# henriChevreux/distillation_trajectories

Measured on AMD Instinct MI355X. Metric: trajectory-timesteps/sec (B×T U-Net fwd) at 16×16 T=50, higher is better.
Workload: dtype f32 (fp32-accurate; convolutions: exact 3-plane bf16 operand split on bf16 MFMA with fp32 accumulate, or native fp32 MFMA, chosen per layer)

## Files before the change

### distillation_trajectories_amd/csrc/dt_conv_strip.hip

```cpp
#include <mutex>
#include <type_traits>

#include "dt_conv_epilogue.h"

namespace dt {

extern __shared__ __attribute__((aligned(16))) __bf16 strip_lds[];

template <int BM, int BN, int KC = 1, int WK = 1>
__global__ __launch_bounds__(256, KC == 1 ? 3 : 2) void conv_strip_bf16x6_kernel(const ConvParams p) {
  constexpr int WN = WK > 1 ? BN / 64 : (BM == 256 ? 1 : 2), WM = 4 / (WN * WK), NT = 256;
  constexpr int MI = BM / (32 * WM), NI = BN / (32 * WN);
  constexpr int KW = KC / WK;
  static_assert(KC % WK == 0 && MI * 32 * WM == BM && NI * 32 * WN == BN && (WK == 1 || (MI == 2 && NI == 2)), "wave layout");
  constexpr int PLANE_B = BN * 16, STAGE_B = 3 * PLANE_B;
  constexpr int AP = BM == 256 ? 3 : (KC == 4 ? 1 : 2);
  const int halo = strip_halo(p.W, BM);
  const int R = BM + 2 * halo;
  const int RZ = (R + 7) & ~7;
  const int PLANE_A = (RZ + 8) * 16;
  __bf16 *As = strip_lds;
  __bf16 *Bs = strip_lds + KC * 3 * PLANE_A;

  const int tid = threadIdx.x, lane = tid & 63;
  const int wave = __builtin_amdgcn_readfirstlane(tid >> 6);
  const int wk = wave % WK, wm = (wave / WK) / WN, wn = (wave / WK) % WN;
  const int half = lane >> 5, l31 = lane & 31;
  const int m0 = blockIdx.x * BM, n0 = blockIdx.y * BN;
  const int HW = p.H * p.W;
  const int CC = p.cin_p >> 4;

  bool s_in[AP], s_ok[AP], s_core[AP];
  int s_off[AP], s_off2[AP], s_offb[AP], s_lds[AP];
#pragma unroll
  for (int i = 0; i < AP; ++i) {
    const int item = tid + i * NT;
    const int srow = item >> 1, hh = item & 1;
    const int m = m0 - halo + srow;
    s_in[i] = item < 2 * R;
    s_ok[i] = s_in[i] && m >= 0 && m < p.M;
    s_core[i] = s_ok[i] && srow >= halo && srow < halo + BM;
    const int mm = s_ok[i] ? m : 0;
    s_off[i] = mm * p.cin_p + hh * 8;
    s_off2[i] = mm * p.cin2_p + hh * 8;
    s_offb[i] = mm * p.b_stride + hh * 8;
    s_lds[i] = srow * 16 + ((hh ^ ((srow >> 3) & 1)) << 3);
  }
  constexpr bool B_ALL = WK > 1 && BN * 4 == NT;
  constexpr int NB = B_ALL ? KC * 3 / 2 : KC * 3, SB = B_ALL ? 2 : 1;
  static_assert(!B_ALL || (KC * 3) % 2 == 0, "weight staging");
  const bool b_thread = B_ALL || tid < BN * 2;
  const int bt = B_ALL ? (tid & (BN * 2 - 1)) : tid, bsub = B_ALL ? tid / (BN * 2) : 0;
  const size_t w_plane = (size_t)p.n_p * 16;
  const __bf16 *wbase = reinterpret_cast<const __bf16 *>(p.w) + (size_t)n0 * 16 + bt * 8 + bsub * w_plane;
  const __bf16 *wbase2 = reinterpret_cast<const __bf16 *>(p.w2) + (size_t)n0 * 16 + bt * 8 + bsub * w_plane;
  const int b_lds = bsub * PLANE_B + bt * 8;

  int a_row[MI];
  unsigned a_mask[MI];
#pragma unroll
  for (int mi = 0; mi < MI; ++mi) {
    const int row_i = wm * (MI * 32) + mi * 32 + l31;
    const int m = m0 + row_i;
    a_row[mi] = row_i + halo;
    unsigned mask = 0;
    if (m < p.M) {
      const int rem = m % HW;
      const int y = rem / p.W, x = rem - y * p.W;
#pragma unroll
      for (int t = 0; t < 9; ++t) {
        const int yy = y + t / 3 - 1, xx = x + t % 3 - 1;
        if (yy >= 0 && yy < p.H && xx >= 0 && xx < p.W) mask |= 1u << t;
      }
    }
    a_mask[mi] = mask;
  }
  int b_frag[NI];
#pragma unroll
  for (int ni = 0; ni < NI; ++ni) {
    const int row = wn * (NI * 32) + ni * 32 + l31;
    b_frag[ni] = row * 16 + ((half ^ ((row >> 3) & 1)) << 3);
  }

  f32x16 acc[MI][NI];
#pragma unroll
  for (int mi = 0; mi < MI; ++mi)
#pragma unroll
    for (int ni = 0; ni < NI; ++ni)
#pragma unroll
      for (int r = 0; r < 16; ++r) acc[mi][ni][r] = 0.f;

  const int n_main = (CC + p.splits * KC - 1) / (p.splits * KC);
  const int cc0 = blockIdx.z * n_main * KC;
  const int CC2 = p.cin2_p >> 4;
  const int n_chunks = n_main + (p.in2 ? (CC2 + KC - 1) / KC : 0);

  f32x4 sa0[KC][AP], sa1[KC][AP];
  u32x4 rb[NB];
  auto load_strip = [&](int ch) __attribute__((always_inline)) {
#pragma unroll
    for (int kk = 0; kk < KC; ++kk)
#pragma unroll
    for (int i = 0; i < AP; ++i) {
      sa0[kk][i] = f32x4{0.f, 0.f, 0.f, 0.f}; sa1[kk][i] = sa0[kk][i];
      if (ch < n_main) {
        const int cc = cc0 + ch * KC + kk;
        if (s_ok[i] && cc < CC) {
          const float *src = (p.in_b && cc >= p.cc_a) ? p.in_b + s_offb[i] + (cc - p.cc_a) * 16 : p.in + s_off[i] + cc * 16;
          sa0[kk][i] = *reinterpret_cast<const f32x4 *>(src);
          sa1[kk][i] = *reinterpret_cast<const f32x4 *>(src + 4);
        }
      } else if (s_core[i] && (ch - n_main) * KC + kk < CC2) {
        const int c2 = (ch - n_main) * KC + kk;
        const float *src = (p.in2_b && c2 >= p.cc_a) ? p.in2_b + s_offb[i] + (c2 - p.cc_a) * 16 : p.in2 + s_off2[i] + c2 * 16;
        sa0[kk][i] = *reinterpret_cast<const f32x4 *>(src);
        sa1[kk][i] = *reinterpret_cast<const f32x4 *>(src + 4);
      }
    }
  };
  auto write_strip = [&]() __attribute__((always_inline)) {
#pragma unroll
    for (int kk = 0; kk < KC; ++kk)
#pragma unroll
    for (int i = 0; i < AP; ++i)
      if (s_in[i]) {
        bf16x8 p1, p2, p3;
        split8(sa0[kk][i], sa1[kk][i], p1, p2, p3);
        __bf16 *A = As + kk * 3 * PLANE_A;
        *reinterpret_cast<bf16x8 *>(A + s_lds[i]) = p1;
        *reinterpret_cast<bf16x8 *>(A + PLANE_A + s_lds[i]) = p2;
        *reinterpret_cast<bf16x8 *>(A + 2 * PLANE_A + s_lds[i]) = p3;
      }
  };
  const size_t tap_stride = (size_t)p.ccw * 3 * w_plane, group_stride = (size_t)KC * 3 * w_plane;
  const __bf16 *wrun = wbase + (size_t)cc0 * 3 * w_plane;
  enum { ADV_NONE = 0, ADV_TAP, ADV_GROUP, ADV_SKIP0, ADV_SKIP };
  auto load_b = [&](int adv) __attribute__((always_inline)) {
    if (adv == ADV_TAP) wrun += tap_stride;
    else if (adv == ADV_GROUP) wrun = wrun - 8 * tap_stride + group_stride;
    else if (adv == ADV_SKIP0) wrun = wbase2;
    else if (adv == ADV_SKIP) wrun += group_stride;
    if (b_thread) {
#pragma unroll
      for (int i = 0; i < NB; ++i)
        rb[i] = *reinterpret_cast<const u32x4 *>(wrun + (SB * i) * w_plane);
    }
  };
  auto write_b = [&](int stage) __attribute__((always_inline)) {
    if (b_thread) {
      __bf16 *B = Bs + stage * KC * STAGE_B;
#pragma unroll
      for (int i = 0; i < NB; ++i) *reinterpret_cast<u32x4 *>(B + (SB * i) * PLANE_B + b_lds) = rb[i];
    }
  };

  constexpr bool DB = WK > 1;
  bf16x8 fbn[KW][NI][3];
  auto load_bd = [&](int adv) __attribute__((always_inline)) {
    if (adv == ADV_TAP) wrun += tap_stride;
    else if (adv == ADV_GROUP) wrun = wrun - 8 * tap_stride + group_stride;
    else if (adv == ADV_SKIP0) wrun = wbase2;
    else if (adv == ADV_SKIP) wrun += group_stride;
    const __bf16 *wt = wrun - (bt * 8 + bsub * w_plane);
#pragma unroll
    for (int kw = 0; kw < KW; ++kw)
#pragma unroll
      for (int ni = 0; ni < NI; ++ni)
#pragma unroll
        for (int pl = 0; pl < 3; ++pl)
          fbn[kw][ni][pl] = *reinterpret_cast<const bf16x8 *>(wt + ((wk * KW + kw) * 3 + pl) * w_plane + b_frag[ni]);
  };

  load_strip(0);
  if (DB) load_bd(ADV_NONE); else load_b(ADV_NONE);
  if (tid < 48 * KC) *reinterpret_cast<u32x4 *>(As + (tid >> 4) * PLANE_A + RZ * 16 + (tid & 15) * 8) = u32x4{0u, 0u, 0u, 0u};
  write_strip();
  if (!DB) write_b(0);
  __syncthreads();

  int step = 0;
  bool stage_next_strip = true;
  auto do_step = [&](auto TT, int ch, bool first_tap, bool last_tap, bool next_chunk, int adv) __attribute__((always_inline)) {
    constexpr int tt = decltype(TT)::value;
    const bool more = !last_tap || next_chunk;
    if (first_tap && next_chunk && stage_next_strip) load_strip(ch + 1);
    bf16x8 fbc[KW][NI][3];
    if (DB) {
#pragma unroll
      for (int kw = 0; kw < KW; ++kw)
#pragma unroll
        for (int ni = 0; ni < NI; ++ni)
#pragma unroll
          for (int pl = 0; pl < 3; ++pl) fbc[kw][ni][pl] = fbn[kw][ni][pl];
      if (more) load_bd(adv);
    } else if (more) load_b(adv);
    {
      int wv = p.W;
      asm volatile("" : "+s"(wv));
      const int shift = (tt / 3 - 1) * wv + (tt % 3 - 1);
      int a_e[MI];
#pragma unroll
      for (int mi = 0; mi < MI; ++mi) {
        int row0 = a_row[mi];
        asm volatile("" : "+v"(row0));
        const int srow = row0 + shift;
        const int lrow = ((a_mask[mi] >> tt) & 1u) ? srow : RZ + (srow & 7);
        a_e[mi] = lrow * 16 + ((half ^ ((srow >> 3) & 1)) << 3);
      }
#pragma unroll
      for (int kw = 0; kw < KW; ++kw) {
        const int kk = wk * KW + kw;
        const __bf16 *A = As + kk * 3 * PLANE_A;
        const __bf16 *B = Bs + ((step & 1) * KC + kk) * STAGE_B;
        bf16x8 fb[NI][3];
#pragma unroll
        for (int ni = 0; ni < NI; ++ni)
#pragma unroll
          for (int pl = 0; pl < 3; ++pl)
            fb[ni][pl] = DB ? fbc[kw][ni][pl] : *reinterpret_cast<const bf16x8 *>(B + pl * PLANE_B + b_frag[ni]);
#pragma unroll
        for (int mi = 0; mi < MI; ++mi) {
          bf16x8 fa[3];
#pragma unroll
          for (int pl = 0; pl < 3; ++pl)
            fa[pl] = *reinterpret_cast<const bf16x8 *>(A + pl * PLANE_A + a_e[mi]);
#pragma unroll
          for (int ni = 0; ni < NI; ++ni) {
            f32x16 c = acc[mi][ni];
            c = __builtin_amdgcn_mfma_f32_32x32x16_bf16(fa[2], fb[ni][0], c, 0, 0, 0);
            c = __builtin_amdgcn_mfma_f32_32x32x16_bf16(fa[1], fb[ni][1], c, 0, 0, 0);
            c = __builtin_amdgcn_mfma_f32_32x32x16_bf16(fa[0], fb[ni][2], c, 0, 0, 0);
            c = __builtin_amdgcn_mfma_f32_32x32x16_bf16(fa[1], fb[ni][0], c, 0, 0, 0);
            c = __builtin_amdgcn_mfma_f32_32x32x16_bf16(fa[0], fb[ni][1], c, 0, 0, 0);
            c = __builtin_amdgcn_mfma_f32_32x32x16_bf16(fa[0], fb[ni][0], c, 0, 0, 0);
            acc[mi][ni] = c;
          }
        }
      }
    }
    if (!DB && more) write_b((step + 1) & 1);
    const bool restage = last_tap && next_chunk && stage_next_strip;
    if (restage) {
      __syncthreads();
      write_strip();
    }
    if (!DB || restage) __syncthreads();
    ++step;
  };

  constexpr bool DIRECT = MI * KW <= 2 && KC >= 2;
  f32x4 ga0[KW][MI][2], ga1[KW][MI][2];
  const int n_skip = p.in2 ? (CC2 + KC - 1) / KC : 0;
  auto load_a = [&](f32x4 (&g)[KW][MI][2], int s2) __attribute__((always_inline)) {
#pragma unroll
    for (int kw = 0; kw < KW; ++kw)
#pragma unroll
      for (int mi = 0; mi < MI; ++mi) {
        const int c2 = s2 * KC + wk * KW + kw;
        const int m = m0 + wm * (MI * 32) + mi * 32 + l31;
        g[kw][mi][0] = f32x4{0.f, 0.f, 0.f, 0.f}; g[kw][mi][1] = g[kw][mi][0];
        if (m < p.M && c2 < CC2) {
          const float *src = (p.in2_b && c2 >= p.cc_a) ? p.in2_b + (size_t)m * p.b_stride + (c2 - p.cc_a) * 16 + half * 8
                                                       : p.in2 + (size_t)m * p.cin2_p + c2 * 16 + half * 8;
          g[kw][mi][0] = *reinterpret_cast<const f32x4 *>(src);
          g[kw][mi][1] = *reinterpret_cast<const f32x4 *>(src + 4);
        }
      }
  };
  auto skip_step = [&](f32x4 (&g)[KW][MI][2], int s2) __attribute__((always_inline)) {
    const bool more = s2 + 1 < n_skip;
    bf16x8 fbc[KW][NI][3];
    if (DB) {
#pragma unroll
      for (int kw = 0; kw < KW; ++kw)
#pragma unroll
        for (int ni = 0; ni < NI; ++ni)
#pragma unroll
          for (int pl = 0; pl < 3; ++pl) fbc[kw][ni][pl] = fbn[kw][ni][pl];
      if (more) load_bd(ADV_SKIP);
    } else if (more) load_b(ADV_SKIP);
#pragma unroll
    for (int kw = 0; kw < KW; ++kw) {
      const int kk = wk * KW + kw;
      const __bf16 *B = Bs + ((step & 1) * KC + kk) * STAGE_B;
      bf16x8 fb[NI][3];
#pragma unroll
      for (int ni = 0; ni < NI; ++ni)
#pragma unroll
        for (int pl = 0; pl < 3; ++pl) fb[ni][pl] = DB ? fbc[kw][ni][pl] : *reinterpret_cast<const bf16x8 *>(B + pl * PLANE_B + b_frag[ni]);
#pragma unroll
      for (int mi = 0; mi < MI; ++mi) {
        bf16x8 fa[3];
        split8(g[kw][mi][0], g[kw][mi][1], fa[0], fa[1], fa[2]);
#pragma unroll
        for (int ni = 0; ni < NI; ++ni) {
          f32x16 c = acc[mi][ni];
          c = __builtin_amdgcn_mfma_f32_32x32x16_bf16(fa[2], fb[ni][0], c, 0, 0, 0);
          c = __builtin_amdgcn_mfma_f32_32x32x16_bf16(fa[1], fb[ni][1], c, 0, 0, 0);
          c = __builtin_amdgcn_mfma_f32_32x32x16_bf16(fa[0], fb[ni][2], c, 0, 0, 0);
          c = __builtin_amdgcn_mfma_f32_32x32x16_bf16(fa[1], fb[ni][0], c, 0, 0, 0);
          c = __builtin_amdgcn_mfma_f32_32x32x16_bf16(fa[0], fb[ni][1], c, 0, 0, 0);
          c = __builtin_amdgcn_mfma_f32_32x32x16_bf16(fa[0], fb[ni][0], c, 0, 0, 0);
          acc[mi][ni] = c;
        }
      }
    }
    if (s2 + 2 < n_skip) load_a(g, s2 + 2);
    if (!DB) {
      if (more) write_b((step + 1) & 1);
      __syncthreads();
    }
    ++step;
  };

  const int prio_grp = ((blockIdx.x + gridDim.x * (blockIdx.y + gridDim.y * blockIdx.z)) >> 8) & 1;
  const bool use_prio = gridDim.x * gridDim.y * gridDim.z <= 512;
  for (int ch = 0; ch < n_main; ++ch) {
    if (use_prio) {
      if ((ch ^ prio_grp) & 1) __builtin_amdgcn_s_setprio(1);
      else __builtin_amdgcn_s_setprio(0);
    }
    const bool next_chunk = ch + 1 < ((WK > 1 && p.in2) ? n_main : n_chunks);
    if (DIRECT && WK == 1 && p.in2 && ch + 1 == n_main) {
      stage_next_strip = false;
      load_a(ga0, 0);
      if (n_skip > 1) load_a(ga1, 1);
    }
    do_step(std::integral_constant<int, 0>{}, ch, true, false, next_chunk, ADV_TAP);
    do_step(std::integral_constant<int, 1>{}, ch, false, false, next_chunk, ADV_TAP);
    do_step(std::integral_constant<int, 2>{}, ch, false, false, next_chunk, ADV_TAP);
    do_step(std::integral_constant<int, 3>{}, ch, false, false, next_chunk, ADV_TAP);
    do_step(std::integral_constant<int, 4>{}, ch, false, false, next_chunk, ADV_TAP);
    do_step(std::integral_constant<int, 5>{}, ch, false, false, next_chunk, ADV_TAP);
    do_step(std::integral_constant<int, 6>{}, ch, false, false, next_chunk, ADV_TAP);
    do_step(std::integral_constant<int, 7>{}, ch, false, false, next_chunk, ADV_TAP);
    do_step(std::integral_constant<int, 8>{}, ch, false, true, next_chunk, ch + 1 < n_main ? ADV_GROUP : ADV_SKIP0);
    if (ch + 1 == n_main && p.in2) {
      if constexpr (WK == 1) {
        conv_midpoint<MI, NI>(p, acc, n0, wn, l31);
      } else {
        constexpr int P = BN + 4, COPY = WM * 32 * P;
        float *red = reinterpret_cast<float *>(strip_lds);
#pragma unroll
        for (int mi = 0; mi < MI; ++mi) {
          if (mi || DB) __syncthreads();
#pragma unroll
          for (int ni = 0; ni < NI; ++ni)
#pragma unroll
            for (int r = 0; r < 16; ++r)
              red[wk * COPY + (wm * 32 + 4 * half + (r & 3) + 8 * (r >> 2)) * P + wn * (NI * 32) + ni * 32 + l31] = acc[mi][ni][r];
          __syncthreads();
#pragma unroll
          for (int ni = 0; ni < NI; ++ni)
#pragma unroll
            for (int r = 0; r < 16; ++r) {
              const float *src = red + (wm * 32 + 4 * half + (r & 3) + 8 * (r >> 2)) * P + wn * (NI * 32) + ni * 32 + l31;
              float v = src[0];
#pragma unroll
              for (int c = 1; c < WK; ++c) v += src[c * COPY];
              acc[mi][ni][r] = wk == 0 ? v : 0.f;
            }
        }
        if (wk == 0) conv_midpoint<MI, NI>(p, acc, n0, wn, l31);
        __syncthreads();
        if (DB) load_bd(ADV_SKIP0); else load_b(ADV_SKIP0);
        if (DIRECT) {
          load_a(ga0, 0);
          if (n_skip > 1) load_a(ga1, 1);
        } else {
          load_strip(n_main);
          if (tid < 48 * KC) *reinterpret_cast<u32x4 *>(As + (tid >> 4) * PLANE_A + RZ * 16 + (tid & 15) * 8) = u32x4{0u, 0u, 0u, 0u};
          write_strip();
        }
        if (!DB) write_b(step & 1);
        __syncthreads();
      }
    }
  }
  __builtin_amdgcn_s_setprio(0);
  if (DIRECT) {
    for (int s2 = 0; s2 < n_skip; s2 += 2) {
      skip_step(ga0, s2);
      if (s2 + 1 < n_skip) skip_step(ga1, s2 + 1);
    }
  } else {
    for (int ch = n_main; ch < n_chunks; ++ch)
      do_step(std::integral_constant<int, 4>{}, ch, true, true, ch + 1 < n_chunks, ADV_SKIP);
  }
  conv_epilogue<MI, NI, WM, WK>(p, acc, reinterpret_cast<float *>(strip_lds), m0, n0, wm, wn, half, l31, wk);
}

int launch_conv_strip(const ConvParams &p_in, hipStream_t s) {
  ConvParams p = p_in;
  const int bm = p.bm, bn = p.bn, kind = p.kind;
  const int kc = strip_kc(kind, bm, bn);
  dim3 grid((p.M + bm - 1) / bm, p.n_p / bn, p.splits);
  size_t lds = strip_lds_bytes(p.W, bm, bn, kind);
  p.dup_stage2 = 0;
  if (p.n_dup == 2 && p.pool_out) {
    const size_t rows1 = bm == 256 || kc == 4 || (kind == KIND_STRIPK && bm == 128) ? 128 : 64;
    const size_t rows2 = bm == 256 ? 128 : (bm == 128 ? 64 : 32);
    const size_t need = (rows1 + (kind == KIND_STRIPK ? rows2 : rows1)) * (bn + 4) * sizeof(float);
    if (need <= strip_lds_limit(kind)) {
      p.dup_stage2 = 1;
      if (need > lds) lds = need;
    }
  }
  if (kind != KIND_STRIP) {
    static std::once_flag attr_once;
    static int attr_status = DT_OK;
    std::call_once(attr_once, [] {
      const void *fns[8] = {reinterpret_cast<const void *>(&conv_strip_bf16x6_kernel<64, 128, 2, 2>),
                            reinterpret_cast<const void *>(&conv_strip_bf16x6_kernel<64, 64, 4, 4>),
                            reinterpret_cast<const void *>(&conv_strip_bf16x6_kernel<128, 64, 2, 2>),
                            reinterpret_cast<const void *>(&conv_strip_bf16x6_kernel<256, 64, 2>),
                            reinterpret_cast<const void *>(&conv_strip_bf16x6_kernel<128, 128, 2>),
                            reinterpret_cast<const void *>(&conv_strip_bf16x6_kernel<128, 64, 2>),
                            reinterpret_cast<const void *>(&conv_strip_bf16x6_kernel<64, 128, 2>),
                            reinterpret_cast<const void *>(&conv_strip_bf16x6_kernel<64, 64, 2>)};
      for (const void *f : fns) {
        const hipError_t e = hipFuncSetAttribute(f, hipFuncAttributeMaxDynamicSharedMemorySize, 98304);
        if (e != hipSuccess) attr_status = (int)e;
      }
    });
    if (attr_status != DT_OK) return attr_status;
    if (kind == KIND_STRIPK && bn == 128) conv_strip_bf16x6_kernel<64, 128, 2, 2><<<grid, 256, lds, s>>>(p);
    else if (kind == KIND_STRIPK && bm == 64) conv_strip_bf16x6_kernel<64, 64, 4, 4><<<grid, 256, lds, s>>>(p);
    else if (kind == KIND_STRIPK) conv_strip_bf16x6_kernel<128, 64, 2, 2><<<grid, 256, lds, s>>>(p);
    else if (bm == 256) conv_strip_bf16x6_kernel<256, 64, 2><<<grid, 256, lds, s>>>(p);
    else if (bm == 128 && bn == 128) conv_strip_bf16x6_kernel<128, 128, 2><<<grid, 256, lds, s>>>(p);
    else if (bm == 128) conv_strip_bf16x6_kernel<128, 64, 2><<<grid, 256, lds, s>>>(p);
    else if (bn == 128) conv_strip_bf16x6_kernel<64, 128, 2><<<grid, 256, lds, s>>>(p);
    else conv_strip_bf16x6_kernel<64, 64, 2><<<grid, 256, lds, s>>>(p);
    DT_LAUNCH_CHECK();
    return DT_OK;
  }
  if (bm == 256) conv_strip_bf16x6_kernel<256, 64><<<grid, 256, lds, s>>>(p);
  else if (bm == 128 && bn == 128) conv_strip_bf16x6_kernel<128, 128><<<grid, 256, lds, s>>>(p);
  else if (bm == 128) conv_strip_bf16x6_kernel<128, 64><<<grid, 256, lds, s>>>(p);
  else if (bn == 128) conv_strip_bf16x6_kernel<64, 128><<<grid, 256, lds, s>>>(p);
  else conv_strip_bf16x6_kernel<64, 64><<<grid, 256, lds, s>>>(p);
  DT_LAUNCH_CHECK();
  return DT_OK;
}

}
```

Before: 353,700.

## Double-buffer A strip in split-K strip conv, staging one item per tap

For the split-K (WK>1) strip convolution variants, the A input strip becomes a two-buffer ring in LDS. Next-chunk strip items are loaded and split into bf16 planes one item per tap, interleaved with the MFMA work, instead of loaded at the first tap and written behind an extra barrier at chunk end. The weight pointer is recomputed per tile without per-thread offsets, and the split-K reduction for the skip input moves out of the chunk loop. The cost is roughly double the A-strip LDS footprint, with the dynamic LDS cap raised to 160KB for these kernels, which can lower occupancy.

```diff
diff --git a/distillation_trajectories_amd/csrc/dt_conv_strip.hip b/distillation_trajectories_amd/csrc/dt_conv_strip.hip
--- a/distillation_trajectories_amd/csrc/dt_conv_strip.hip
+++ b/distillation_trajectories_amd/csrc/dt_conv_strip.hip
@@ -132,6 +132,32 @@
         *reinterpret_cast<bf16x8 *>(A + 2 * PLANE_A + s_lds[i]) = p3;
       }
   };
+  constexpr int NS = KC * AP;
+  f32x4 st0, st1;
+  auto load_item = [&](auto J, int ch) __attribute__((always_inline)) {
+    constexpr int kk = decltype(J)::value / AP, i = decltype(J)::value % AP;
+    const int cc = cc0 + ch * KC + kk, ccl = cc < CC ? cc : CC - 1;
+    const bool ok = s_ok[i] && cc < CC, from_b = p.in_b && ccl >= p.cc_a;
+    const float *base = from_b ? p.in_b + (ccl - p.cc_a) * 16 : p.in + ccl * 16;
+    unsigned off = s_off[i], offb = s_offb[i];
+    asm volatile("" : "+v"(off), "+v"(offb));
+    const float *src = base + (from_b ? offb : off);
+    const f32x4 v0 = *reinterpret_cast<const f32x4 *>(src), v1 = *reinterpret_cast<const f32x4 *>(src + 4);
+    const f32x4 z = {0.f, 0.f, 0.f, 0.f};
+    st0 = ok ? v0 : z;
+    st1 = ok ? v1 : z;
+  };
+  auto write_item = [&](auto J, int buf) __attribute__((always_inline)) {
+    constexpr int kk = decltype(J)::value / AP, i = decltype(J)::value % AP;
+    if (s_in[i]) {
+      bf16x8 p1, p2, p3;
+      split8(st0, st1, p1, p2, p3);
+      __bf16 *A = As + (buf * KC + kk) * 3 * PLANE_A;
+      *reinterpret_cast<bf16x8 *>(A + s_lds[i]) = p1;
+      *reinterpret_cast<bf16x8 *>(A + PLANE_A + s_lds[i]) = p2;
+      *reinterpret_cast<bf16x8 *>(A + 2 * PLANE_A + s_lds[i]) = p3;
+    }
+  };
   const size_t tap_stride = (size_t)p.ccw * 3 * w_plane, group_stride = (size_t)KC * 3 * w_plane;
   const __bf16 *wrun = wbase + (size_t)cc0 * 3 * w_plane;
   enum { ADV_NONE = 0, ADV_TAP, ADV_GROUP, ADV_SKIP0, ADV_SKIP };
@@ -155,25 +181,31 @@
   };
 
   constexpr bool DB = WK > 1;
+  static_assert(!DB || NS <= 8, "strip items staged one per tap");
   bf16x8 fbn[KW][NI][3];
+  const __bf16 *wtile = DB ? reinterpret_cast<const __bf16 *>(p.w) + (size_t)n0 * 16 + (size_t)cc0 * 3 * w_plane : nullptr;
   auto load_bd = [&](int adv) __attribute__((always_inline)) {
-    if (adv == ADV_TAP) wrun += tap_stride;
-    else if (adv == ADV_GROUP) wrun = wrun - 8 * tap_stride + group_stride;
-    else if (adv == ADV_SKIP0) wrun = wbase2;
-    else if (adv == ADV_SKIP) wrun += group_stride;
-    const __bf16 *wt = wrun - (bt * 8 + bsub * w_plane);
+    if (adv == ADV_TAP) wtile += tap_stride;
+    else if (adv == ADV_GROUP) wtile = wtile - 8 * tap_stride + group_stride;
+    else if (adv == ADV_SKIP0) wtile = reinterpret_cast<const __bf16 *>(p.w2) + (size_t)n0 * 16;
+    else if (adv == ADV_SKIP) wtile += group_stride;
 #pragma unroll
     for (int kw = 0; kw < KW; ++kw)
 #pragma unroll
-      for (int ni = 0; ni < NI; ++ni)
+      for (int ni = 0; ni < NI; ++ni) {
+        unsigned off = b_frag[ni];
+        asm volatile("" : "+v"(off));
 #pragma unroll
         for (int pl = 0; pl < 3; ++pl)
-          fbn[kw][ni][pl] = *reinterpret_cast<const bf16x8 *>(wt + ((wk * KW + kw) * 3 + pl) * w_plane + b_frag[ni]);
+          fbn[kw][ni][pl] = *reinterpret_cast<const bf16x8 *>(wtile + ((wk * KW + kw) * 3 + pl) * w_plane + off);
+      }
   };
 
   load_strip(0);
   if (DB) load_bd(ADV_NONE); else load_b(ADV_NONE);
-  if (tid < 48 * KC) *reinterpret_cast<u32x4 *>(As + (tid >> 4) * PLANE_A + RZ * 16 + (tid & 15) * 8) = u32x4{0u, 0u, 0u, 0u};
+  if constexpr (DB) {
+    for (int z = tid; z < 96 * KC; z += NT) *reinterpret_cast<u32x4 *>(As + (z >> 4) * PLANE_A + RZ * 16 + (z & 15) * 8) = u32x4{0u, 0u, 0u, 0u};
+  } else if (tid < 48 * KC) *reinterpret_cast<u32x4 *>(As + (tid >> 4) * PLANE_A + RZ * 16 + (tid & 15) * 8) = u32x4{0u, 0u, 0u, 0u};
   write_strip();
   if (!DB) write_b(0);
   __syncthreads();
@@ -183,9 +215,9 @@
   auto do_step = [&](auto TT, int ch, bool first_tap, bool last_tap, bool next_chunk, int adv) __attribute__((always_inline)) {
     constexpr int tt = decltype(TT)::value;
     const bool more = !last_tap || next_chunk;
-    if (first_tap && next_chunk && stage_next_strip) load_strip(ch + 1);
+    if (!DB && first_tap && next_chunk && stage_next_strip) load_strip(ch + 1);
     bf16x8 fbc[KW][NI][3];
-    if (DB) {
+    if constexpr (DB) {
 #pragma unroll
       for (int kw = 0; kw < KW; ++kw)
 #pragma unroll
@@ -193,6 +225,8 @@
 #pragma unroll
           for (int pl = 0; pl < 3; ++pl) fbc[kw][ni][pl] = fbn[kw][ni][pl];
       if (more) load_bd(adv);
+      if constexpr (tt >= 1 && tt <= NS) write_item(std::integral_constant<int, tt - 1 < NS ? tt - 1 : 0>{}, (ch + 1) & 1);
+      if constexpr (tt < NS) load_item(std::integral_constant<int, tt < NS ? tt : 0>{}, ch + 1);
     } else if (more) load_b(adv);
     {
       int wv = p.W;
@@ -210,7 +244,7 @@
 #pragma unroll
       for (int kw = 0; kw < KW; ++kw) {
         const int kk = wk * KW + kw;
-        const __bf16 *A = As + kk * 3 * PLANE_A;
+        const __bf16 *A = As + ((DB ? (ch & 1) * KC : 0) + kk) * 3 * PLANE_A;
         const __bf16 *B = Bs + ((step & 1) * KC + kk) * STAGE_B;
         bf16x8 fb[NI][3];
 #pragma unroll
@@ -240,7 +274,7 @@
     }
     if (!DB && more) write_b((step + 1) & 1);
     const bool restage = last_tap && next_chunk && stage_next_strip;
-    if (restage) {
+    if (!DB && restage) {
       __syncthreads();
       write_strip();
     }
@@ -335,47 +369,46 @@
     do_step(std::integral_constant<int, 6>{}, ch, false, false, next_chunk, ADV_TAP);
     do_step(std::integral_constant<int, 7>{}, ch, false, false, next_chunk, ADV_TAP);
     do_step(std::integral_constant<int, 8>{}, ch, false, true, next_chunk, ch + 1 < n_main ? ADV_GROUP : ADV_SKIP0);
-    if (ch + 1 == n_main && p.in2) {
-      if constexpr (WK == 1) {
-        conv_midpoint<MI, NI>(p, acc, n0, wn, l31);
-      } else {
-        constexpr int P = BN + 4, COPY = WM * 32 * P;
-        float *red = reinterpret_cast<float *>(strip_lds);
-#pragma unroll
-        for (int mi = 0; mi < MI; ++mi) {
-          if (mi || DB) __syncthreads();
-#pragma unroll
-          for (int ni = 0; ni < NI; ++ni)
-#pragma unroll
-            for (int r = 0; r < 16; ++r)
-              red[wk * COPY + (wm * 32 + 4 * half + (r & 3) + 8 * (r >> 2)) * P + wn * (NI * 32) + ni * 32 + l31] = acc[mi][ni][r];
-          __syncthreads();
-#pragma unroll
-          for (int ni = 0; ni < NI; ++ni)
-#pragma unroll
-            for (int r = 0; r < 16; ++r) {
-              const float *src = red + (wm * 32 + 4 * half + (r & 3) + 8 * (r >> 2)) * P + wn * (NI * 32) + ni * 32 + l31;
-              float v = src[0];
-#pragma unroll
-              for (int c = 1; c < WK; ++c) v += src[c * COPY];
-              acc[mi][ni][r] = wk == 0 ? v : 0.f;
-            }
+    if constexpr (WK == 1) {
+      if (ch + 1 == n_main && p.in2) conv_midpoint<MI, NI>(p, acc, n0, wn, l31);
+    }
+  }
+  if constexpr (WK > 1) if (p.in2) {
+    constexpr int P = BN + 4, COPY = WM * 32 * P;
+    float *red = reinterpret_cast<float *>(strip_lds);
+#pragma unroll
+    for (int mi = 0; mi < MI; ++mi) {
+      if (mi || DB) __syncthreads();
+#pragma unroll
+      for (int ni = 0; ni < NI; ++ni)
+#pragma unroll
+        for (int r = 0; r < 16; ++r)
+          red[wk * COPY + (wm * 32 + 4 * half + (r & 3) + 8 * (r >> 2)) * P + wn * (NI * 32) + ni * 32 + l31] = acc[mi][ni][r];
+      __syncthreads();
+#pragma unroll
+      for (int ni = 0; ni < NI; ++ni)
+#pragma unroll
+        for (int r = 0; r < 16; ++r) {
+          const float *src = red + (wm * 32 + 4 * half + (r & 3) + 8 * (r >> 2)) * P + wn * (NI * 32) + ni * 32 + l31;
+          float v = src[0];
+#pragma unroll
+          for (int c = 1; c < WK; ++c) v += src[c * COPY];
+          acc[mi][ni][r] = wk == 0 ? v : 0.f;
         }
-        if (wk == 0) conv_midpoint<MI, NI>(p, acc, n0, wn, l31);
-        __syncthreads();
-        if (DB) load_bd(ADV_SKIP0); else load_b(ADV_SKIP0);
-        if (DIRECT) {
-          load_a(ga0, 0);
-          if (n_skip > 1) load_a(ga1, 1);
-        } else {
-          load_strip(n_main);
-          if (tid < 48 * KC) *reinterpret_cast<u32x4 *>(As + (tid >> 4) * PLANE_A + RZ * 16 + (tid & 15) * 8) = u32x4{0u, 0u, 0u, 0u};
-          write_strip();
-        }
-        if (!DB) write_b(step & 1);
-        __syncthreads();
-      }
-    }
+    }
+    if (wk == 0) conv_midpoint<MI, NI>(p, acc, n0, wn, l31);
+    __syncthreads();
+    if (DB) load_bd(ADV_SKIP0); else load_b(ADV_SKIP0);
+    if (DIRECT) {
+      load_a(ga0, 0);
+      if (n_skip > 1) load_a(ga1, 1);
+    } else {
+      load_strip(n_main);
+      if (tid < 48 * KC) *reinterpret_cast<u32x4 *>(As + (tid >> 4) * PLANE_A + RZ * 16 + (tid & 15) * 8) = u32x4{0u, 0u, 0u, 0u};
+      write_strip();
+    }
+    if (!DB) write_b(step & 1);
+    __syncthreads();
   }
   __builtin_amdgcn_s_setprio(0);
   if (DIRECT) {
@@ -396,6 +429,11 @@
   const int kc = strip_kc(kind, bm, bn);
   dim3 grid((p.M + bm - 1) / bm, p.n_p / bn, p.splits);
   size_t lds = strip_lds_bytes(p.W, bm, bn, kind);
+  if (kind == KIND_STRIPK) {
+    const int rows = ((bm + 2 * strip_halo(p.W, bm) + 7) & ~7) + 8;
+    const size_t ring = (size_t)2 * kc * 3 * rows * 16 * sizeof(__bf16);
+    if (ring > lds) lds = ring;
+  }
   p.dup_stage2 = 0;
   if (p.n_dup == 2 && p.pool_out) {
     const size_t rows1 = bm == 256 || kc == 4 || (kind == KIND_STRIPK && bm == 128) ? 128 : 64;
@@ -418,8 +456,8 @@
                             reinterpret_cast<const void *>(&conv_strip_bf16x6_kernel<128, 64, 2>),
                             reinterpret_cast<const void *>(&conv_strip_bf16x6_kernel<64, 128, 2>),
                             reinterpret_cast<const void *>(&conv_strip_bf16x6_kernel<64, 64, 2>)};
-      for (const void *f : fns) {
-        const hipError_t e = hipFuncSetAttribute(f, hipFuncAttributeMaxDynamicSharedMemorySize, 98304);
+      for (int i = 0; i < 8; ++i) {
+        const hipError_t e = hipFuncSetAttribute(fns[i], hipFuncAttributeMaxDynamicSharedMemorySize, i < 3 ? 163840 : 98304);
         if (e != hipSuccess) attr_status = (int)e;
       }
     });
```

New measurement: 361,400, median of 6. 1.02x the previous value.
